# thu-ml/SageAttention

Measured on AMD Instinct MI355X. Metric: attention TFLOPS (causal, hd=128), kernel-only, as published by the reference, higher is better.
Workload: dtype int8 QK^T + fp8(e4m3) PV, fp32 accumulate

## Files before the change

sageattention_amd/csrc/sage_attn_kernel.h:

```cpp
#pragma once
#include "sage_common.h"
#include "sage_kernels.h"
#include "sage_attn_parts.h"
#include "sage_quant_math.h"
#include "sage_work_order.h"
#include <atomic>
#include <climits>
#include <cstdlib>
#include <type_traits>

#ifndef SAGE_ABL
#define SAGE_ABL 0
#endif
#ifndef SAGE_DIAG_PIPE
#define SAGE_DIAG_PIPE 1
#endif
#ifndef SAGE_KARG_PREFETCH
#define SAGE_KARG_PREFETCH 1
#endif
#ifndef SAGE_TAIL_PIPE
#define SAGE_TAIL_PIPE 1
#endif
#ifndef SAGE_KSEL
#define SAGE_KSEL 1
#endif
#ifndef SAGE_ATTN_TRACE
#define SAGE_ATTN_TRACE 0
#endif

#define SAGE_MIN_WAVES(D, MASK) ((MASK) != 0 ? 2 : ((D) == 64 ? 3 : 2))

#define SAGE_SCALE2_FOLD(d0, d1, s0, s1, c0, c1, m) "v_fma_f32 " d0 ", " s0 ", " c0 ", -" m "\n\tv_fma_f32 " d1 ", " s1 ", " c1 ", -" m "\n\t"
#define SAGE_SCALE2_EXACT(d0, d1, s0, s1, c0, c1, m) "v_add_f32 " d0 ", 0xbe22f983, " s0 "\n\tv_add_f32 " d1 ", 0xbe22f983, " s1 "\n\t" \
                                                      "v_fma_f32 " d0 ", " d0 ", " c0 ", -" m "\n\tv_fma_f32 " d1 ", " d1 ", " c1 ", -" m "\n\t"

#define SAGE_RENAME_S() do { const v4i z4_ = {0, 0, 0, 0};                                                                   \
        asm volatile("s_nop 15\n\ts_nop 7\n\tv_mfma_i32_32x32x32_i8 %0, %2, %2, %3\n\tv_mfma_i32_32x32x32_i8 %1, %2, %2, %4\n\t"     \
                     "s_nop 15\n\ts_nop 7" : "=&v"(sA[0]), "=&v"(sA[1]) : "v"(z4_), "v"(sB[0]), "v"(sB[1])); } while (0)

namespace sage {

constexpr int kHwregModeFp16Ovfl = 1 | (23 << 6) | (0 << 11);


template <int D, bool PV_FP8, int NH> struct TileCfg {
    static constexpr int KT = BLKK * NH;
    static constexpr int K_TILE_BYTES = KT * D;
    static constexpr int V_ROW_BYTES = PV_FP8 ? 64 : 128;
    static constexpr int V_IMG_BYTES = D * V_ROW_BYTES;
    static constexpr int STAGE_BYTES = K_TILE_BYTES + NH * V_IMG_BYTES;
    static constexpr int O_BYTES = BLKQ * D * 2;
    static constexpr int NSTAGE = 3;
    static constexpr int LDS_BYTES = (NSTAGE * STAGE_BYTES > O_BYTES) ? NSTAGE * STAGE_BYTES : O_BYTES;
    static constexpr int KSTEPS = D / 32;
    static constexpr int DT = D / 32;
};

__device__ __forceinline__ int crow(int r, int g) { return (r & 3) + 8 * (r >> 2) + 4 * g; }

constexpr int kSUnitLog2 = 26;
__device__ __forceinline__ float sfl(int x) { return __int_as_float(x) - __int_as_float(0x3E22F983); }
__device__ __forceinline__ v16i mfma_i8_first(v4i a, v4i b)
{
    v16i d;
    asm("s_nop 1\n\tv_mfma_i32_32x32x32_i8 %0, %1, %2, 0x3e22f983" : "=&v"(d) : "v"(a), "v"(b));
    return d;
}

#if SAGE_ATTN_TRACE
#define SAGE_TSTAMP(i) do { if (wave == 0) { unsigned long long t_; \
    asm volatile("s_memrealtime %0\n\ts_waitcnt lgkmcnt(0)" : "=s"(t_) :: "memory"); ttrace[i] = (unsigned)t_; } } while (0)
#else
#define SAGE_TSTAMP(i) do { } while (0)
#endif

template <int D, bool PV_FP8, bool CAUSAL, bool KTHREAD, bool TWO_LEVEL, int NH, int MASK = 0, int QF = 0, bool SFOLD = true, bool CPERS = false,
          bool VROWS = false, bool SEED = false>
__global__ void __launch_bounds__(256, SAGE_MIN_WAVES(D, MASK))
sage_attn_kernel(const AttnParams p_arg)
{
    typedef const __attribute__((address_space(4))) AttnParams *kparams_t;
    const kparams_t kp0 = (kparams_t)__builtin_amdgcn_kernarg_segment_ptr();
    const __attribute__((address_space(4))) AttnParams &p = *kp0;
    (void)p_arg;
#if SAGE_KARG_PREFETCH
    static_assert(sizeof(AttnParams) > 0x180, "prefetch offsets lie inside the parameter block");
    {
        unsigned t0, t1, t2, t3, t4, t5, t6;
        asm volatile("s_load_dword %0, %7, 0x0\n\ts_load_dword %1, %7, 0x40\n\ts_load_dword %2, %7, 0x80\n\ts_load_dword %3, %7, 0xc0\n\t"
                     "s_load_dword %4, %7, 0x100\n\ts_load_dword %5, %7, 0x140\n\ts_load_dword %6, %7, 0x180\n\ts_waitcnt lgkmcnt(0)"
                     : "=&s"(t0), "=&s"(t1), "=&s"(t2), "=&s"(t3), "=&s"(t4), "=&s"(t5), "=&s"(t6) : "s"(kp0) : "memory");
    }
#endif
    using C = TileCfg<D, PV_FP8, NH>;
    constexpr int KT = C::KT;
    constexpr int NS = 2 * NH;
    static_assert(!SEED || (PV_FP8 && KTHREAD && TWO_LEVEL && !SFOLD && MASK == 0 && (QF == 1 || QF == 2) && !CPERS && !VROWS),
                  "the seeded split: FP8 PV, fused per-thread Q, exact score form, dense");
    extern __shared__ __attribute__((aligned(16))) unsigned char smem[];

    const int wave_s = __builtin_amdgcn_readfirstlane((int)threadIdx.x >> 6);
#if SAGE_ATTN_TRACE
    __shared__ unsigned ttrace[16];
#endif
    constexpr bool PERS_OK = (!CAUSAL || CPERS) && MASK == 0;
    const bool pers = PERS_OK && p.sched != nullptr;
    __shared__ int s_ticket[2];
    int tpar = 0;
    int bid = blockIdx.x;
    unsigned next_k_v = 0;
    bool have_next = false, own_empty = false;
    auto kpl = [&]() -> kparams_t { kparams_t k = kp0; asm volatile("" : "+s"(k)); return k; };
    auto my_queue = [&]() -> int { return 4 * (int)(__builtin_amdgcn_s_getreg((3 << 11) | 20) & 7u) + (int)((blockIdx.x >> 3) & 3u); };
    auto logical_grid = [&]() -> int {
        const __attribute__((address_space(4))) AttnParams &pl = *kpl();
        int n = pl.nwg;
        if (pl.cu_q != nullptr && pl.work_items != nullptr) {
            typedef const __attribute__((address_space(4))) int *cint_p;
            const cint_p hdr = (cint_p)pl.work_hdr;
            n = 8 * (hdr[3] * ((hdr[0] + 7) >> 3) + (pl.Hq >> 3) * hdr[0]);
        }
        return n;
    };
    auto resolve_ticket = [&]() -> int {
        const int nwg_l = logical_grid();
        const int sched_first = gridDim.x >> 5;
        const int my_q = my_queue(), my_xcd = my_q >> 2;
        unsigned *const sched = kpl()->sched;
        if (have_next) {
            have_next = false;
            const int i = 32 * ((int)__builtin_amdgcn_readfirstlane(next_k_v) + sched_first) + 8 * (my_q & 3) + my_xcd;
            if (i < nwg_l) return i;
            own_empty = true;
        }
        int lane_o = (int)__builtin_amdgcn_mbcnt_hi(~0u, __builtin_amdgcn_mbcnt_lo(~0u, 0u));
        asm volatile("" : "+v"(lane_o));
        for (int attempt = 0; attempt < 4; attempt++) {
            const int q = lane_o & 31, x = q >> 2, s8x = 8 * (q & 3) + x;
            const unsigned c = lane_o < 32 ? __hip_atomic_load(sched + 32 * q, __ATOMIC_RELAXED, __HIP_MEMORY_SCOPE_AGENT) : 0u;
            const int cnt = nwg_l > s8x ? (nwg_l - s8x + 31) >> 5 : 0;
            int left = cnt - sched_first - (int)c;
            left = left < (1 << 24) ? left : (1 << 24) - 1;
            unsigned key = (lane_o < 32 && left > 0) ? ((x == my_xcd ? 1u : 0u) << 30) | ((unsigned)left << 5) | (unsigned)q : 0u;
#pragma unroll
            for (int m = 32; m >= 1; m >>= 1) { const unsigned o = __shfl_xor(key, m); key = o > key ? o : key; }
            key = __builtin_amdgcn_readfirstlane(key);
            if (key == 0u) return -1;
            const int bq = (int)(key & 31u);
            unsigned kv = 0;
            if (lane_o == 0) kv = __hip_atomic_fetch_add(sched + 32 * bq, 1u, __ATOMIC_RELAXED, __HIP_MEMORY_SCOPE_AGENT);
            const int i = 32 * ((int)__builtin_amdgcn_readfirstlane(kv) + sched_first) + 8 * (bq & 3) + (bq >> 2);
            if (i < nwg_l) return i;
        }
        return -1;
    };
    while (bid >= 0) {
    next_k_v = 0;
    do {
    kparams_t kp = kp0;
    if constexpr (PERS_OK) asm volatile("" : "+s"(kp));
    const __attribute__((address_space(4))) AttnParams &p = *kp;
    int lane_v = (int)__builtin_amdgcn_mbcnt_hi(~0u, __builtin_amdgcn_mbcnt_lo(~0u, 0u));
    if constexpr (PERS_OK) asm volatile("v_mbcnt_lo_u32_b32 %0, -1, 0\n\tv_mbcnt_hi_u32_b32 %0, -1, %0" : "=v"(lane_v));
    const int lane = lane_v;
    const int wave = wave_s;
    [[maybe_unused]] const int tid = wave * 64 + lane;
    int n = lane & 31;
    int g = lane >> 5;
    SAGE_TSTAMP(0);
    __builtin_amdgcn_s_setreg(kHwregModeFp16Ovfl, 1);

    const int nqblk = p.nqblk;
    int b, h, hk, qblk;
    if (p.cu_q != nullptr && p.work_items != nullptr) {
        typedef const __attribute__((address_space(4))) int *cint_p;
        const cint_p hdr = (cint_p)p.work_hdr;
        const int nitems = hdr[0];
        const WorkOrder wo = {hdr[1], hdr[2], hdr[3]};
        const int nwg = 8 * (wo.left * ((nitems + 7) >> 3) + (p.Hq >> 3) * nitems);
        int qrank;
        if (bid >= nwg || !work_item(wo, bid, nwg, p.Hq, nitems, h, qrank)) break;
        const cint_p items = (cint_p)p.work_items;
        b = items[2 * qrank];
        qblk = items[2 * qrank + 1];
        hk = h / p.group;
    } else if (p.cu_q != nullptr) {
        const int xcd = bid & 7, idx = bid >> 3;
        const int per_unit = nqblk * p.group;
        const int j = idx / per_unit, within = idx - j * per_unit;
        const int u = j * 8 + xcd;
        if (u >= p.B * p.Hkv) break;
        const int r = within / p.group, hg = within - r * p.group;
        qblk = nqblk - 1 - r;
        const int bs = u / p.Hkv;
        hk = u - bs * p.Hkv;
        b = p.seq_order != nullptr ? p.seq_order[bs] : bs;
        h = hk * p.group + hg;
    } else {
        int bh, qrank;
        const WorkOrder wo = {CAUSAL ? p.order_group : 0, p.order_fold, p.order_left};
        if (!work_item(wo, bid, pers ? p.nwg : (int)gridDim.x, p.B * p.Hq, nqblk, bh, qrank)) break;
        qblk = nqblk - 1 - qrank;
        b = bh / p.Hq;
        h = bh - b * p.Hq;
        hk = h / p.group;
    }

    int Lq = p.Lq, Lk = p.Lk;
    long q_off, k_off, o_off;
    long v_tile0, v_tstride;
    const float *qs_ptr, *ks_ptr;
    int qs_stride, ks_tstride;
    if (p.cu_q != nullptr) {
        typedef const __attribute__((address_space(4))) int *cint_p;
        const int bu = __builtin_amdgcn_readfirstlane(b);
        const int q0 = ((cint_p)p.cu_q)[bu], k0 = ((cint_p)p.cu_k)[bu], q1 = ((cint_p)p.cu_q)[bu + 1], k1 = ((cint_p)p.cu_k)[bu + 1];
        const int ks0 = ((cint_p)p.cu_ks)[bu];
        Lq = q1 - q0;
        Lk = k1 - k0;
        if (qblk * BLKQ >= Lq) break;
        q_off = (long)q0 * p.q_sl + (long)h * p.q_sh;
        k_off = (long)k0 * p.k_sl + (long)hk * p.k_sh;
        o_off = (long)q0 * p.o_sl + (long)h * p.o_sh;
        v_tile0 = (long)ks0 * p.Hkv + hk;
        v_tstride = p.Hkv;
        qs_ptr = QF == 0 ? p.q_scale + ((long)((cint_p)p.cu_qs)[bu] + qblk) * p.Hq + h : nullptr;
        qs_stride = 0;
        ks_ptr = p.k_scale + (long)ks0 * p.Hkv + hk;
        ks_tstride = p.Hkv;
    } else if constexpr (SEED) {
        const int hk0 = hk / p.kv_split, kc0 = p.kv_base + (hk - hk0 * p.kv_split) * Lk;
        const long bh0 = (long)b * (p.Hkv / p.kv_split) + hk0;
        q_off = (long)b * p.q_sb + (long)(hk0 * p.group + (h - hk * p.group)) * p.q_sh;
        k_off = (long)b * p.k_sb + (long)hk0 * p.k_sh + (long)kc0 * p.k_sl;
        o_off = (long)b * p.o_sb + (long)h * p.o_sh;
        v_tile0 = bh0 * (p.nks >> 2) + (kc0 >> 6);
        v_tstride = 1;
        qs_ptr = nullptr;
        qs_stride = 0;
        ks_ptr = p.k_scale + bh0 * p.nks + (kc0 >> 6) * 4;
        ks_tstride = 4;
    } else {
        const int hq = p.kv_split > 1 ? (hk / p.kv_split) * p.group + (h - hk * p.group) : h;
        q_off = (long)b * p.q_sb + (long)hq * p.q_sh;
        k_off = (long)b * p.k_sb + (long)hk * p.k_sh;
        o_off = (long)b * p.o_sb + (long)h * p.o_sh;
        const int ntk = (Lk + BLKK - 1) / BLKK;
        v_tile0 = ((long)b * p.Hkv + hk) * ntk;
        v_tstride = 1;
        qs_ptr = p.q_scale + ((long)b * p.Hq + h) * p.nqs + (long)qblk * p.qs_per_blk;
        qs_stride = 1;
        ks_ptr = p.k_scale + ((long)b * p.Hkv + hk) * p.nks;
        ks_tstride = KTHREAD ? 4 : 1;
    }

    SAGE_TSTAMP(1);
    const int row0 = qblk * BLKQ + wave * 32;
    int my_row = row0 + n;
    const int kchunk0 = SEED ? (CAUSAL ? p.kv_base + (hk % p.kv_split) * Lk : 0)
                             : ((CAUSAL && p.kv_split > 1 && p.cu_q == nullptr) ? (hk % p.kv_split) * Lk : 0);
    const int crow0 = row0 - kchunk0;
    int cmy_row = my_row - kchunk0;
    const int ntk_all = (Lk + BLKK - 1) / BLKK;
    int n_iters = (Lk + KT - 1) / KT;
    if (CAUSAL) {
        int lim = (qblk * BLKQ + BLKQ - kchunk0 + KT - 1) / KT;
        lim = lim > 0 ? lim : 0;
        n_iters = lim < n_iters ? lim : n_iters;
    }

    v4i qf[C::KSTEPS];
    float qsc;
    const unsigned char *kbase = reinterpret_cast<const unsigned char *>(p.k) + k_off;
    static_assert(!VROWS || (!PV_FP8 && MASK == 0), "V rows in place: FP16 PV, unmasked, dense launches");
    const unsigned char *vbase = reinterpret_cast<const unsigned char *>(p.v) + (VROWS ? 2 * ((long)b * p.v_sb + (long)hk * p.v_sh) : 0L);
    constexpr int CPR = D / 16;
    constexpr int KP = C::K_TILE_BYTES / 1024, VP = C::V_IMG_BYTES / 1024;
    unsigned koff[KP / 4];
#pragma unroll
    for (int i = 0; i < KP / 4; i++) {
        const int e = (wave * (KP / 4) + i) * 64 + lane;
        const int row = e / CPR, phys = e % CPR;
        koff[i] = (unsigned)(row * (int)p.k_sl + swz_chunk<D>(row, phys) * 16);
    }
    constexpr int CPRV = D / 8;
    constexpr int RPP = 64 / CPRV;
    [[maybe_unused]] unsigned voffr = 0;
    if constexpr (VROWS) {
        const int row = lane / CPRV, phys = lane % CPRV;
        const int logical = D == 128 ? (phys ^ ((row & 3) << 2)) : phys;
        voffr = (unsigned)(row * (int)p.v_sl * 2 + logical * 16);
    }
    typedef __attribute__((address_space(3))) unsigned char *lds_bytes;
    [[maybe_unused]] int vr_off[C::DT];
    if constexpr (VROWS) {
        const int s16 = lane & 15, hgrp = (lane >> 4) & 1;
#pragma unroll
        for (int dt = 0; dt < C::DT; dt++)
            vr_off[dt] = (4 * g + (s16 >> 2)) * (D * 2) + (D == 128 ? (dt ^ (s16 >> 2)) : dt) * 64 + 32 * hgrp + 8 * (s16 & 3);
    }
    auto v_frag = [&](const unsigned char *vs, int dt, int c) -> v4i {
        if constexpr (VROWS) {
            typedef short v4s __attribute__((ext_vector_type(4)));
            typedef short v8s __attribute__((ext_vector_type(8)));
            typedef __attribute__((address_space(3))) v4s *lds_v4s;
            const lds_bytes a0 = (lds_bytes)vs + vr_off[dt];
            const v4s lo = __builtin_amdgcn_ds_read_tr16_b64_v4i16((lds_v4s)(a0 + 16 * c * (D * 2)));
            const v4s hi = __builtin_amdgcn_ds_read_tr16_b64_v4i16((lds_v4s)(a0 + (16 * c + 8) * (D * 2)));
            return __builtin_bit_cast(v4i, (v8s)__builtin_shufflevector(lo, hi, 0, 1, 2, 3, 4, 5, 6, 7));
        } else {
            const int drow = dt * 32 + n;
            return *reinterpret_cast<const v4i *>(vs + drow * 128 + swz_chunk<128>(drow, 4 * g + c) * 16);
        }
    };
    int lane_g = lane;
    auto issue_loads = [&](int it, int buf) {
        unsigned char *ks = smem + buf * C::STAGE_BYTES;
        unsigned char *vs = ks + C::K_TILE_BYTES;
        const unsigned char *kt = kbase + (long)it * KT * p.k_sl;
        if (it * KT + KT <= Lk) {
#pragma unroll
            for (int i = 0; i < KP / 4; i++) {
                const int pc = wave * (KP / 4) + i;
                __builtin_amdgcn_global_load_lds((const __attribute__((address_space(1))) void *)(kt + koff[i]),
                                                 (__attribute__((address_space(3))) void *)(ks + pc * 1024), 16, 0, 0);
            }
        } else {
#pragma unroll
            for (int i = 0; i < KP / 4; i++) {
                const int pc = wave * (KP / 4) + i;
                const int e = pc * 64 + lane_g;
                const int row = e / CPR, phys = e % CPR;
                int key = it * KT + row;
                key = key < Lk ? key : Lk - 1;
                const unsigned char *src = kbase + (long)key * p.k_sl + swz_chunk<D>(row, phys) * 16;
                __builtin_amdgcn_global_load_lds((const __attribute__((address_space(1))) void *)src,
                                                 (__attribute__((address_space(3))) void *)(ks + pc * 1024), 16, 0, 0);
            }
        }
#pragma unroll
        for (int hh = 0; hh < NH; hh++) {
            int tv = it * NH + hh;
            tv = tv < ntk_all ? tv : ntk_all - 1;
            if constexpr (VROWS) {
#pragma unroll
                for (int i = 0; i < VP / 4; i++) {
                    const int pc = wave * (VP / 4) + i;
                    int tok = tv * BLKK + pc * RPP + lane_g / CPRV;
                    tok = tok < Lk ? tok : Lk - 1;
                    const int row = pc * RPP + lane_g / CPRV, phys = lane_g % CPRV;
                    const int logical = D == 128 ? (phys ^ ((row & 3) << 2)) : phys;
                    __builtin_amdgcn_global_load_lds((const __attribute__((address_space(1))) void *)(vbase + (long)tok * p.v_sl * 2 + logical * 16),
                                                     (__attribute__((address_space(3))) void *)(vs + hh * C::V_IMG_BYTES + pc * 1024), 16, 0, 0);
                }
            } else {
            const unsigned char *vt = vbase + (v_tile0 + (long)tv * v_tstride) * (long)C::V_IMG_BYTES;
#pragma unroll
            for (int i = 0; i < VP / 4; i++) {
                const int pc = wave * (VP / 4) + i;
                __builtin_amdgcn_global_load_lds((const __attribute__((address_space(1))) void *)(vt + pc * 1024 + lane_g * 16),
                                                 (__attribute__((address_space(3))) void *)(vs + hh * C::V_IMG_BYTES + pc * 1024), 16, 0, 0);
            }
            }
        }
    };

    v16f o[C::DT];
#pragma unroll
    for (int dt = 0; dt < C::DT; dt++)
#pragma unroll
        for (int i = 0; i < 16; i++) o[dt][i] = 0.0f;
    float m_run = kNegBig, l_run = 0.0f;
    constexpr float OFF = PV_FP8 ? kFp8Offset : 0.0f;

    typedef const __attribute__((address_space(4))) float *cfloat_p;
    const cfloat_p ks_c = (cfloat_p)(ks_ptr);
    float ksc[NH][2];
    auto load_kscales = [&](int it, float (&dst)[NH][2]) {
#pragma unroll
        for (int hh = 0; hh < NH; hh++) {
            int tk = it * NH + hh;
            tk = tk < ntk_all ? tk : ntk_all - 1;
            const long tb = (long)(tk >> p.ks_shift) * ks_tstride;
            if (KTHREAD) {
                const float s0 = ks_c[tb], s1 = ks_c[tb + 1], s2 = ks_c[tb + 2], s3 = ks_c[tb + 3];
                dst[hh][0] = g ? s2 : s0;
                dst[hh][1] = g ? s3 : s1;
            } else {
                dst[hh][0] = dst[hh][1] = ks_c[tb];
            }
        }
    };
    constexpr int NSTAGE = C::NSTAGE;
    constexpr int DMA_PER_TILE = KP / 4 + NH * (VP / 4);
    auto ring_wait = [&](bool younger_in_flight) {
        if (younger_in_flight) asm volatile("s_waitcnt vmcnt(%0)" ::"n"(DMA_PER_TILE) : "memory");
        else asm volatile("s_waitcnt vmcnt(0)" ::: "memory");
        __builtin_amdgcn_s_barrier();
    };
    if (n_iters > 0) {
        load_kscales(0, ksc);
        issue_loads(0, 0);
    }
    if (n_iters > 1) issue_loads(1, 1);
    if constexpr (QF == 0) {
        const int8_t *qrow = reinterpret_cast<const int8_t *>(p.q) + q_off + (long)my_row * p.q_sl;
        const bool ok = my_row < Lq;
#pragma unroll
        for (int ks = 0; ks < C::KSTEPS; ks++) {
            v4i z = {0, 0, 0, 0};
            qf[ks] = ok ? *reinterpret_cast<const v4i *>(qrow + 32 * ks + 16 * g) : z;
        }
        int slot;
        const int rin = wave * 32 + n;
        if (p.q_gran == QG_PER_BLOCK) slot = 0;
        else if (p.q_gran == QG_PER_WARP32) slot = rin >> 5;
        else if (p.q_gran == QG_PER_WARP16) slot = rin >> 4;
        else if (p.q_gran == QG_PER_THREAD16) slot = (rin >> 4) * 8 + (rin & 7);
        else slot = (rin >> 5) * 8 + (rin & 7);
        qsc = qs_ptr[slot * qs_stride];
    } else {
        constexpr int QDT = (QF == 1 || QF == 3) ? DT_F16 : DT_BF16;
        constexpr bool QBLOCK = QF >= 3;
        const float premul = QBLOCK ? p.q_premul : 1.0f;
        const uint16_t *qrow = reinterpret_cast<const uint16_t *>(p.q) + q_off + (long)my_row * p.q_sl;
        const bool ok = my_row < Lq;
        float x[C::KSTEPS][16];
        float amax = 0.0f;
#pragma unroll
        for (int ks = 0; ks < C::KSTEPS; ks++) {
            v4u raw[2] = {{0u, 0u, 0u, 0u}, {0u, 0u, 0u, 0u}};
            if (ok) {
                raw[0] = *reinterpret_cast<const v4u *>(qrow + 32 * ks + 16 * g);
                raw[1] = *reinterpret_cast<const v4u *>(qrow + 32 * ks + 16 * g + 8);
            }
#pragma unroll
            for (int j = 0; j < 16; j++) {
                const unsigned w = raw[j >> 3][(j & 7) >> 1];
                float f = ld16<QDT>((uint16_t)((j & 1) ? (w >> 16) : (w & 0xffffu)));
                if constexpr (QBLOCK) f *= premul;
                x[ks][j] = f;
                amax = fmaxf(amax, fabsf(f));
            }
        }
        if constexpr (QBLOCK) {
            amax = fmaxf(amax, __shfl_xor(amax, 1));
            amax = fmaxf(amax, __shfl_xor(amax, 2));
            amax = fmaxf(amax, __shfl_xor(amax, 4));
        }
        amax = fmaxf(amax, __shfl_xor(amax, 8));
        amax = fmaxf(amax, __shfl_xor(amax, 16));
        amax = fmaxf(amax, __shfl_xor(amax, 32));
        if constexpr (QBLOCK) {
            __shared__ float q_amax[4];
            if (lane == 0) q_amax[wave] = amax;
            asm volatile("s_waitcnt lgkmcnt(0)" ::: "memory");
            __builtin_amdgcn_s_barrier();
            amax = fmaxf(fmaxf(q_amax[0], q_amax[1]), fmaxf(q_amax[2], q_amax[3]));
        }
        const float sc = quant_scale(amax, QBLOCK ? QS_TRITON : QS_TRITON_THREAD);
        const float y = quant_recip(sc);
        qsc = sc;
#pragma unroll
        for (int ks = 0; ks < C::KSTEPS; ks++) {
            int q8[16];
#pragma unroll
            for (int j = 0; j < 16; j++) q8[j] = QBLOCK ? quant_round_triton(x[ks][j], sc, y) : quant_round_triton_nz(x[ks][j], sc, y);
#pragma unroll
            for (int w = 0; w < 4; w++) qf[ks][w] = (int)pack_int8x4(q8[4 * w], q8[4 * w + 1], q8[4 * w + 2], q8[4 * w + 3]);
        }
    }

    if constexpr (SEED) {
        if (my_row < Lq) {
            const int hk0 = hk / p.kv_split;
            const long gl = (long)p.group * Lq;
            const float *sm = p.seed_max + ((long)b * (p.Hkv / p.kv_split) + hk0) * p.seed_chunks * gl + (long)(h - hk * p.group) * Lq + my_row;
            const int c_end = p.seed_first + (hk - hk0 * p.kv_split);
            for (int c = 0; c < c_end; c++) m_run = fmaxf(m_run, sm[c * gl]);
        }
    }
    SAGE_TSTAMP(2);
    ring_wait(n_iters > 1);
    SAGE_TSTAMP(3);

    int cur = 0;
    auto tile_iter = [&](const int it) {
        const bool more = (it + 1) < n_iters;
        const bool more2 = (it + 2) < n_iters;
        const int nxt = (cur + 1 == NSTAGE) ? 0 : cur + 1;
        float ksc_next[NH][2];
        if (more) load_kscales(it + 1, ksc_next);
        if (more2) issue_loads(it + 2, (nxt + 1 == NSTAGE) ? 0 : nxt + 1);

        int nact = 0;
#pragma unroll
        for (int hh = 0; hh < NH; hh++) {
            const int key0 = it * KT + hh * BLKK;
            if (key0 < Lk && (!CAUSAL || key0 <= crow0 + 31)) nact = hh + 1;
        }
        float mk[MASK ? NS : 1][16];
        bool skip_tile = false;
        if constexpr (MASK != 0) {
            const unsigned char *mbase = reinterpret_cast<const unsigned char *>(p.mask);
            const long mrow = (long)b * p.m_sb + (long)h * p.m_sh + (long)my_row * p.m_sq;
            int anytrue = 0;
#pragma unroll
            for (int sb = 0; sb < NS; sb++)
#pragma unroll
                for (int i = 0; i < 16; i++) {
                    const int key = it * KT + sb * 32 + crow(i, g);
                    const bool inb = (my_row < Lq) && (key < Lk);
                    float add = -1.0e6f;
                    if (inb) {
                        const long idx = mrow + (long)key * p.m_sk;
                        if (MASK == 1) { const bool t = mbase[idx] != 0; add = t ? 0.0f : -1.0e6f; anytrue |= (int)t; }
                        else if (MASK == 2) add = f16_to_f32(reinterpret_cast<const uint16_t *>(mbase)[idx]);
                        else add = bf16_to_f32(reinterpret_cast<const uint16_t *>(mbase)[idx]);
                    }
                    mk[sb][i] = add;
                }
            if (MASK == 1) skip_tile = !__syncthreads_or(anytrue);
        }
        if (nact > 0 && !skip_tile) {
            const unsigned char *ks = smem + cur * C::STAGE_BYTES;
            const unsigned char *vs = ks + C::K_TILE_BYTES;
            const int last_key = it * KT + nact * BLKK - 1;
            const bool full = (MASK == 0) && (nact == NH) && !(CAUSAL && last_key > crow0) && (last_key < Lk);

            v16i s[NS];
#pragma unroll
            for (int sb = 0; sb < NS; sb++) {
#pragma unroll
                for (int i = 0; i < 16; i++) s[sb][i] = 0;
                if (sb < 2 * nact) {
                    const int krow = sb * 32 + n;
#pragma unroll
                    for (int kk = 0; kk < C::KSTEPS; kk++) {
                        const v4i a = *reinterpret_cast<const v4i *>(ks + krow * D + swz_chunk<D>(krow, 2 * kk + g) * 16);
                        s[sb] = kk == 0 ? mfma_i8_first(a, qf[kk]) : __builtin_amdgcn_mfma_i32_32x32x32_i8(a, qf[kk], s[sb], 0, 0, 0);
                    }
                }
            }

            float cs[NH][2];
#pragma unroll
            for (int hh = 0; hh < NH; hh++) {
                cs[hh][0] = __builtin_ldexpf(p.sm_scale_log2 * (qsc * ksc[hh][0]), kSUnitLog2);
                cs[hh][1] = KTHREAD ? __builtin_ldexpf(p.sm_scale_log2 * (qsc * ksc[hh][1]), kSUnitLog2) : cs[hh][0];
            }

            float m_new;
            if (full) {
                float mxc = -INFINITY;
#pragma unroll
                for (int hh = 0; hh < NH; hh++) {
                    int mx0 = INT_MIN, mx1 = INT_MIN;
#pragma unroll
                    for (int u = 0; u < 2; u++)
#pragma unroll
                        for (int i = 0; i < 16; i++) {
                            if (KTHREAD && (i & 2)) mx1 = max(mx1, s[2 * hh + u][i]);
                            else mx0 = max(mx0, s[2 * hh + u][i]);
                        }
                    mxc = fmaxf(mxc, __builtin_fmaf(sfl(mx0), cs[hh][0], -OFF));
                    if (KTHREAD) mxc = fmaxf(mxc, __builtin_fmaf(sfl(mx1), cs[hh][1], -OFF));
                }
                m_new = fmaxf(m_run, pair_max(mxc));
            } else {
                float mx = -INFINITY;
#pragma unroll
                for (int sb = 0; sb < NS; sb++)
#pragma unroll
                    for (int i = 0; i < 16; i++) {
                        if (sb < 2 * nact) {
                            const float cc = cs[sb >> 1][(KTHREAD && (i & 2)) ? 1 : 0];
                            const int key = it * KT + sb * 32 + crow(i, g);
                            const bool ok = (key < Lk) && (!CAUSAL || key <= cmy_row);
                            if constexpr (MASK != 0) mx = fmaxf(mx, (ok ? sfl(s[sb][i]) * cc : 0.0f) + mk[sb][i] - OFF);
                            else mx = fmaxf(mx, ok ? __builtin_fmaf(sfl(s[sb][i]), cc, -OFF) : -INFINITY);
                        }
                    }
                m_new = fmaxf(m_run, pair_max(mx));
            }
            const float alpha = __builtin_amdgcn_exp2f(m_run - m_new);
            m_run = m_new;
            if (!TWO_LEVEL) {
#pragma unroll
                for (int dt = 0; dt < C::DT; dt++)
#pragma unroll
                    for (int i = 0; i < 16; i++) o[dt][i] *= alpha;
            }

            constexpr bool sum_rounded = !PV_FP8 && !TWO_LEVEL;
            constexpr bool GFOLD = PV_FP8 && SFOLD && MASK == 0;
            float rs = 0.0f;
            auto p_chunk = [&](auto masked, auto rnd, int hh, int c, float (&e)[8]) {
                const int sb = 2 * hh + (c >> 1), r0 = (c & 1) * 8;
                [[maybe_unused]] const float mbf0 = GFOLD ? __builtin_fmaf(__int_as_float(0x3E22F983), cs[hh][0], m_new) : 0.0f;
                [[maybe_unused]] const float mbf1 = (GFOLD && KTHREAD) ? __builtin_fmaf(__int_as_float(0x3E22F983), cs[hh][1], m_new) : mbf0;
#pragma unroll
                for (int j = 0; j < 8; j++) {
                    const int i = r0 + j;
                    const float cc = cs[hh][(KTHREAD && (i & 2)) ? 1 : 0];
                    float v;
                    if constexpr (MASK != 0) {
                        const int key = it * KT + sb * 32 + crow(i, g);
                        v = __builtin_amdgcn_exp2f(((key < Lk) ? sfl(s[sb][i]) * cc : 0.0f) + mk[sb][i] - m_new);
                    } else {
                        if constexpr (GFOLD) v = __builtin_amdgcn_exp2f(__builtin_fmaf(__int_as_float(s[sb][i]), cc, -((KTHREAD && (i & 2)) ? mbf1 : mbf0)));
                        else v = __builtin_amdgcn_exp2f(__builtin_fmaf(sfl(s[sb][i]), cc, -m_new));
                        if constexpr (decltype(masked)::value) {
                            const int key = it * KT + sb * 32 + crow(i, g);
                            const bool ok = (sb < 2 * nact) && (key < Lk) && (!CAUSAL || key <= cmy_row);
                            v = ok ? v : 0.0f;
                        }
                    }
                    e[j] = v;
                    if constexpr (decltype(rnd)::value) rs += (float)(_Float16)v;
                    else rs += v;
                }
            };

            if constexpr (PV_FP8) {
                int pw[NH][8];
                auto build_p = [&](auto masked) {
#pragma unroll
                    for (int hh = 0; hh < NH; hh++)
#pragma unroll
                        for (int c = 0; c < 4; c++) {
                            float e[8];
                            p_chunk(masked, std::false_type{}, hh, c, e);
                            int w0 = __builtin_amdgcn_cvt_pk_fp8_f32(e[0], e[1], __float_as_int(e[0]), false);
                            w0 = __builtin_amdgcn_cvt_pk_fp8_f32(e[2], e[3], w0, true);
                            int w1 = __builtin_amdgcn_cvt_pk_fp8_f32(e[4], e[5], __float_as_int(e[4]), false);
                            w1 = __builtin_amdgcn_cvt_pk_fp8_f32(e[6], e[7], w1, true);
                            pw[hh][2 * c] = w0;
                            pw[hh][2 * c + 1] = w1;
                        }
                };
                if (full) build_p(std::false_type{});
                else build_p(std::true_type{});
                l_run = l_run * alpha + rs;
                auto pv = [&](auto fold_tag) {
                    constexpr bool FOLD = decltype(fold_tag)::value;
#pragma unroll
                    for (int dt = 0; dt < C::DT; dt++) {
                        const int drow = dt * 32 + n;
                        v16f acc;
                        if (FOLD) {
#pragma unroll
                            for (int i = 0; i < 16; i++) acc[i] = 0.0f;
                        } else acc = o[dt];
#pragma unroll
                        for (int hh = 0; hh < NH; hh++) {
                            if (hh < nact) {
                                const unsigned char *vr = vs + hh * C::V_IMG_BYTES + drow * 64;
                                const v4u va = *reinterpret_cast<const v4u *>(vr + swz_chunk<64>(drow, 2 * g) * 16);
                                const v4u vb = *reinterpret_cast<const v4u *>(vr + swz_chunk<64>(drow, 2 * g + 1) * 16);
                                const v8i av = {(int)va[0], (int)va[1], (int)va[2], (int)va[3], (int)vb[0], (int)vb[1], (int)vb[2], (int)vb[3]};
                                const v8i bv = {pw[hh][0], pw[hh][1], pw[hh][2], pw[hh][3], pw[hh][4], pw[hh][5], pw[hh][6], pw[hh][7]};
                                acc = __builtin_amdgcn_mfma_scale_f32_32x32x64_f8f6f4(av, bv, acc, 0, 0, 0, 0, 0, 0);
                            }
                        }
                        if (FOLD) {
#pragma unroll
                            for (int i = 0; i < 16; i++) o[dt][i] = __builtin_fmaf(o[dt][i], alpha, acc[i]);
                        } else o[dt] = acc;
                    }
                };
                if constexpr (!TWO_LEVEL) pv(std::false_type{});
                else pv(std::true_type{});
            } else {
                v8h pb[NH][4];
                auto build_p = [&](auto masked, auto rnd) {
#pragma unroll
                    for (int hh = 0; hh < NH; hh++)
#pragma unroll
                        for (int c = 0; c < 4; c++) {
                            float e[8];
                            p_chunk(masked, rnd, hh, c, e);
#pragma unroll
                            for (int j = 0; j < 8; j++) pb[hh][c][j] = (_Float16)e[j];
                        }
                };
                if (full) build_p(std::false_type{}, std::integral_constant<bool, sum_rounded>{});
                else build_p(std::true_type{}, std::integral_constant<bool, sum_rounded>{});
                l_run = l_run * alpha + rs;
                auto pv = [&](auto fold_tag) {
                    constexpr bool FOLD = decltype(fold_tag)::value;
#pragma unroll
                    for (int dt = 0; dt < C::DT; dt++) {
                        v16f acc;
                        if (FOLD) {
#pragma unroll
                            for (int i = 0; i < 16; i++) acc[i] = 0.0f;
                        } else acc = o[dt];
#pragma unroll
                        for (int hh = 0; hh < NH; hh++) {
                            if (hh < nact) {
#pragma unroll
                                for (int c = 0; c < 4; c++) {
                                    const v8h a = __builtin_bit_cast(v8h, v_frag(vs + hh * C::V_IMG_BYTES, dt, c));
                                    acc = __builtin_amdgcn_mfma_f32_32x32x16_f16(a, pb[hh][c], acc, 0, 0, 0);
                                }
                            }
                        }
                        if (FOLD) {
#pragma unroll
                            for (int i = 0; i < 16; i++) o[dt][i] = __builtin_fmaf(o[dt][i], alpha, acc[i]);
                        } else o[dt] = acc;
                    }
                };
                if constexpr (!TWO_LEVEL) pv(std::false_type{});
                else pv(std::true_type{});
            }
        }

        if (more) {
#pragma unroll
            for (int hh = 0; hh < NH; hh++) { ksc[hh][0] = ksc_next[hh][0]; ksc[hh][1] = ksc_next[hh][1]; }
        }
        ring_wait(more2);
        cur = nxt;
    };

    int it = 0;
    if constexpr (MASK == 0) {
        static_assert(NH == 1 && NSTAGE == 3, "the pipelined loops are written for 64-key iterations on the 3-slot ring");
        constexpr bool SIX_BODIES = D == 128 || PV_FP8;
        int n_steady = Lk / KT - 2;
        n_steady = n_steady < n_iters - 2 ? n_steady : n_iters - 2;
        if (CAUSAL) {
            int nd = (qblk * BLKQ - kchunk0) / KT;
            nd = nd > 0 ? nd : 0;
            n_steady = n_steady < nd ? n_steady : nd;
        }
        constexpr bool DIAG_PIPE = CAUSAL && SAGE_DIAG_PIPE && (PV_FP8 || D == 128);
        const bool diag_ok = DIAG_PIPE && (n_steady > 0 ? n_iters - n_steady == 2 : (PV_FP8 && n_iters == 2 && Lk >= 2 * KT));
        constexpr bool TAIL_PIPE = !CAUSAL && SAGE_TAIL_PIPE && (PV_FP8 || D == 128);
        const bool tail_ok = TAIL_PIPE && n_steady == Lk / KT - 2 &&
                             (PV_FP8 ? (n_steady >= 0 && n_iters - n_steady <= (SAGE_TAIL_PIPE == 2 ? 2 : 3)) : (n_steady > 0 && n_iters - n_steady == 2));

        if constexpr (PV_FP8) {
#include "sage_attn_loop_f8.h"
        } else {
#include "sage_attn_loop_f16.h"
        }
    }
    if constexpr (MASK == 0) {
        asm volatile("v_mbcnt_lo_u32_b32 %0, -1, 0\n\tv_mbcnt_hi_u32_b32 %0, -1, %0" : "=v"(lane_g));
        n = lane_g & 31;
        g = lane_g >> 5;
        my_row = row0 + n;
        cmy_row = my_row - kchunk0;
    }
#pragma nounroll
    for (; it < n_iters; it++) tile_iter(it);
    SAGE_TSTAMP(4);
    __syncthreads();
    SAGE_TSTAMP(5);
    if (pers && !own_empty) {
        if (wave == 0 && lane_g == 0) next_k_v = __hip_atomic_fetch_add(kpl()->sched + 32 * my_queue(), 1u, __ATOMIC_RELAXED, __HIP_MEMORY_SCOPE_AGENT);
        have_next = true;
    }

    __builtin_amdgcn_s_setreg(kHwregModeFp16Ovfl, 0);
    const float l_tot = pair_sum(l_run);
    const float inv = l_tot > 0.0f ? __builtin_amdgcn_rcpf(l_tot) : 0.0f;
    if (p.lse != nullptr && g == 0 && my_row < Lq) {
        long lidx = (p.cu_q != nullptr) ? ((long)h * p.lse_sh + p.cu_q[b] + my_row)
                                        : ((long)b * p.Hq + h) * (long)p.Lq + my_row;
        p.lse[lidx] = __builtin_amdgcn_logf(l_tot) + m_run;
    }
    unsigned char *obuf = smem + wave * (32 * D * 2);
    const long vbh = SEED ? (long)b * (p.Hkv / p.kv_split) + hk / p.kv_split : (long)b * p.Hkv + hk;
    const float *vsc = PV_FP8 ? p.v_scale + vbh * D : nullptr;
    const float *vmn = (p.v_mean != nullptr) ? p.v_mean + vbh * D : nullptr;
    v4f sc4[C::DT][4], mn4[C::DT][4];
#pragma unroll
    for (int dt = 0; dt < C::DT; dt++) {
#pragma unroll
        for (int r4 = 0; r4 < 4; r4++) {
            const v4f one = {1.0f, 1.0f, 1.0f, 1.0f};
            sc4[dt][r4] = PV_FP8 ? *reinterpret_cast<const v4f *>(vsc + dt * 32 + 8 * r4 + 4 * g) : one;
        }
        if (vmn != nullptr) {
#pragma unroll
            for (int r4 = 0; r4 < 4; r4++) mn4[dt][r4] = *reinterpret_cast<const v4f *>(vmn + dt * 32 + 8 * r4 + 4 * g);
        } else {
#pragma unroll
            for (int r4 = 0; r4 < 4; r4++) { const v4f z = {0.0f, 0.0f, 0.0f, 0.0f}; mn4[dt][r4] = z; }
        }
    }
#pragma unroll
    for (int dt = 0; dt < C::DT; dt++) {
#pragma unroll
        for (int r4 = 0; r4 < 4; r4++) {
            const int d0 = dt * 32 + 8 * r4 + 4 * g;
            float x[4];
#pragma unroll
            for (int j = 0; j < 4; j++) {
                x[j] = o[dt][4 * r4 + j] * inv;
                if (PV_FP8) x[j] *= sc4[dt][r4][j];
                x[j] += mn4[dt][r4][j];
            }
            if constexpr (SEED) {
                if (my_row < Lq) *reinterpret_cast<v4f *>(reinterpret_cast<float *>(p.o) + o_off + (long)my_row * p.o_sl + d0) = v4f{x[0], x[1], x[2], x[3]};
                continue;
            }
            v2u pk;
            if (p.out_dtype == DT_F16) {
                pk[0] = (unsigned)f32_to_f16_rne(x[0]) | ((unsigned)f32_to_f16_rne(x[1]) << 16);
                pk[1] = (unsigned)f32_to_f16_rne(x[2]) | ((unsigned)f32_to_f16_rne(x[3]) << 16);
            } else {
                pk[0] = (unsigned)f32_to_bf16_rne(x[0]) | ((unsigned)f32_to_bf16_rne(x[1]) << 16);
                pk[1] = (unsigned)f32_to_bf16_rne(x[2]) | ((unsigned)f32_to_bf16_rne(x[3]) << 16);
            }
            const int q8 = d0 >> 2;
            const int Q = (q8 >> 1) ^ (n & 7);
            *reinterpret_cast<v2u *>(obuf + n * (D * 2) + Q * 16 + (q8 & 1) * 8) = pk;
        }
    }
    asm volatile("s_waitcnt lgkmcnt(0)" ::: "memory");
    if constexpr (!SEED) {
        constexpr int LPR = D * 2 / 16;
        constexpr int RPP = 64 / LPR;
        unsigned char *obase = reinterpret_cast<unsigned char *>(p.o) + 2 * o_off;
#pragma unroll
        for (int pass = 0; pass < 32 / RPP; pass++) {
            const int r = pass * RPP + lane_g / LPR, Q = lane_g % LPR;
            const v4u val = *reinterpret_cast<const v4u *>(obuf + r * (D * 2) + (Q ^ (r & 7)) * 16);
            const int grow = row0 + r;
            if (grow < Lq) *reinterpret_cast<v4u *>(obase + 2 * ((long)grow * p.o_sl) + Q * 16) = val;
        }
    }
#if SAGE_ATTN_TRACE
    SAGE_TSTAMP(6);
    asm volatile("s_waitcnt vmcnt(0)" ::: "memory");
    SAGE_TSTAMP(7);
    if (wave == 0 && p.trace != nullptr && bid < p.trace_wgs) {
        if (lane < 8 || lane == 8 || lane >= 13) p.trace[16 * bid + lane] = ttrace[lane];
        if (lane == 9) p.trace[16 * bid + 9] = __builtin_amdgcn_s_getreg((31 << 11) | 4);
        if (lane == 10) p.trace[16 * bid + 10] = __builtin_amdgcn_s_getreg((31 << 11) | 20);
        if (lane == 11) p.trace[16 * bid + 11] = blockIdx.x;
        if (lane == 12) p.trace[16 * bid + 12] = (unsigned)qblk;
    }
#endif
    } while (0);
    if (!pers) break;
    if (wave_s == 0) { const int t = resolve_ticket(); if (__builtin_amdgcn_mbcnt_hi(~0u, __builtin_amdgcn_mbcnt_lo(~0u, 0u)) == 0) s_ticket[tpar] = t; }
    __syncthreads();
    bid = __builtin_amdgcn_readfirstlane(s_ticket[tpar]);
    tpar ^= 1;
    }
    if constexpr (PERS_OK) {
        if (pers && wave_s == 0) {
            unsigned *const sched = kpl()->sched;
            const int lane_x = (int)__builtin_amdgcn_mbcnt_hi(~0u, __builtin_amdgcn_mbcnt_lo(~0u, 0u));
            unsigned gone = 0;
            if (lane_x == 0) gone = __hip_atomic_fetch_add(sched + kAttnSchedDoneWord, 1u, __ATOMIC_ACQ_REL, __HIP_MEMORY_SCOPE_AGENT);
            if ((unsigned)__builtin_amdgcn_readfirstlane(gone) + 1u == gridDim.x) {
                if (lane_x < 32) __hip_atomic_store(sched + 32 * lane_x, 0u, __ATOMIC_RELAXED, __HIP_MEMORY_SCOPE_AGENT);
                if (lane_x == 32) __hip_atomic_store(sched + kAttnSchedDoneWord, 0u, __ATOMIC_RELAXED, __HIP_MEMORY_SCOPE_AGENT);
            }
        }
    }
}

}
```

sageattention_amd/csrc/sage_common.h:

```cpp
#pragma once
#include <hip/hip_runtime.h>
#include <stdint.h>

namespace sage {

typedef int v4i __attribute__((ext_vector_type(4)));
typedef int v8i __attribute__((ext_vector_type(8)));
typedef int v16i __attribute__((ext_vector_type(16)));
typedef float v16f __attribute__((ext_vector_type(16)));
typedef float v4f __attribute__((ext_vector_type(4)));
typedef float v2f __attribute__((ext_vector_type(2)));
typedef _Float16 v8h __attribute__((ext_vector_type(8)));
typedef _Float16 v2h __attribute__((ext_vector_type(2)));
typedef unsigned int v4u __attribute__((ext_vector_type(4)));
typedef unsigned int v2u __attribute__((ext_vector_type(2)));

constexpr int kWave = 64;
constexpr int BLKQ = 128;
constexpr int BLKK = 64;
constexpr float kFp8Offset = 8.807f;
constexpr float kNegBig = -1.0e30f;

enum : int { DT_F16 = 0, DT_BF16 = 1 };

__host__ __device__ inline int pv_token_of_position(int p)
{
    const int g = p >> 5, c = (p >> 3) & 3, j = p & 7;
    return 16 * c + 8 * (j >> 2) + 4 * g + (j & 3);
}

template <int ROW_BYTES>
__host__ __device__ inline int swz_chunk(int row, int chunk)
{
    if constexpr (ROW_BYTES == 128) return chunk ^ ((row >> 1) & 7);
    else if constexpr (ROW_BYTES == 64) return chunk ^ ((row >> 2) & 3);
    else return chunk;
}

__device__ inline float bf16_to_f32(uint16_t b) { return __uint_as_float(((uint32_t)b) << 16); }
__device__ inline uint16_t f32_to_bf16_rne(float f)
{
    uint32_t x = __float_as_uint(f);
    x += 0x7fffu + ((x >> 16) & 1u);
    return (uint16_t)(x >> 16);
}
__device__ inline float f16_to_f32(uint16_t h)
{
    _Float16 v; __builtin_memcpy(&v, &h, 2); return (float)v;
}
__device__ inline uint16_t f32_to_f16_rne(float f)
{
    _Float16 v = (_Float16)f; uint16_t h; __builtin_memcpy(&h, &v, 2); return h;
}
template <int DT> __device__ inline float ld16(uint16_t raw)
{
    if constexpr (DT == DT_F16) return f16_to_f32(raw); else return bf16_to_f32(raw);
}
template <int DT> __device__ inline uint16_t st16(float f)
{
    if constexpr (DT == DT_F16) return f32_to_f16_rne(f); else return f32_to_bf16_rne(f);
}

__device__ inline float pair_max(float x)
{
    auto r = __builtin_amdgcn_permlane32_swap(__float_as_uint(x), __float_as_uint(x), false, false);
    return fmaxf(__uint_as_float(r[0]), __uint_as_float(r[1]));
}
__device__ inline float pair_sum(float x)
{
    auto r = __builtin_amdgcn_permlane32_swap(__float_as_uint(x), __float_as_uint(x), false, false);
    return __uint_as_float(r[0]) + __uint_as_float(r[1]);
}

template <typename IntPtr>
__device__ __forceinline__ void varlen_segment(IntPtr cu, int nseq, int total, int seg, int &t0, int &len)
{
    if (seg < nseq) { t0 = cu[seg]; len = cu[seg + 1] - t0; }
    else if (seg == nseq) { t0 = cu[nseq]; len = total - t0; }
    else { t0 = 0; len = cu[0]; }
    len = len > 0 ? len : 0;
}

}
```

Measured before the change: 1604.

## Trim attention epilogue: prefetch scale factors before barrier, specialize output conversion and stores

Issues the v_scale/v_mean loads before the end-of-loop barrier so their latency overlaps the wait, and replaces __syncthreads with a raw s_barrier. The output conversion is specialized by dtype at compile time, with bf16 using a packed hardware conversion. The global store loop batches its LDS reads and skips per-row bounds checks when the whole tile is in range. The gains are limited to the per-tile epilogue, and the packed bf16 conversion may round differently from the manual RNE on NaN inputs.

```diff
diff --git a/sageattention_amd/csrc/sage_attn_kernel.h b/sageattention_amd/csrc/sage_attn_kernel.h
--- a/sageattention_amd/csrc/sage_attn_kernel.h
+++ b/sageattention_amd/csrc/sage_attn_kernel.h
@@ -23,6 +23,9 @@
 #endif
 #ifndef SAGE_KSEL
 #define SAGE_KSEL 1
+#endif
+#ifndef SAGE_ITEM_TRIM
+#define SAGE_ITEM_TRIM 2
 #endif
 #ifndef SAGE_ATTN_TRACE
 #define SAGE_ATTN_TRACE 0
@@ -758,7 +761,36 @@
 #pragma nounroll
     for (; it < n_iters; it++) tile_iter(it);
     SAGE_TSTAMP(4);
-    __syncthreads();
+    constexpr bool TRIM_EPI = (SAGE_ITEM_TRIM & 2) != 0;
+    const long vbh = SEED ? (long)b * (p.Hkv / p.kv_split) + hk / p.kv_split : (long)b * p.Hkv + hk;
+    const float *vsc = PV_FP8 ? p.v_scale + vbh * D : nullptr;
+    const float *vmn = (p.v_mean != nullptr) ? p.v_mean + vbh * D : nullptr;
+    v4f sc4[C::DT][4], mn4[C::DT][4];
+    auto load_factors = [&]() {
+#pragma unroll
+        for (int dt = 0; dt < C::DT; dt++) {
+#pragma unroll
+            for (int r4 = 0; r4 < 4; r4++) {
+                const v4f one = {1.0f, 1.0f, 1.0f, 1.0f};
+                sc4[dt][r4] = PV_FP8 ? *reinterpret_cast<const v4f *>(vsc + dt * 32 + 8 * r4 + 4 * g) : one;
+            }
+            if (vmn != nullptr) {
+#pragma unroll
+                for (int r4 = 0; r4 < 4; r4++) mn4[dt][r4] = *reinterpret_cast<const v4f *>(vmn + dt * 32 + 8 * r4 + 4 * g);
+            } else {
+#pragma unroll
+                for (int r4 = 0; r4 < 4; r4++) { const v4f z = {0.0f, 0.0f, 0.0f, 0.0f}; mn4[dt][r4] = z; }
+            }
+        }
+    };
+    if constexpr (TRIM_EPI) {
+        load_factors();
+        asm volatile("s_waitcnt lgkmcnt(0)" ::: "memory");
+        __builtin_amdgcn_s_barrier();
+        asm volatile("" ::: "memory");
+    } else {
+        __syncthreads();
+    }
     SAGE_TSTAMP(5);
     if (pers && !own_empty) {
         if (wave == 0 && lane_g == 0) next_k_v = __hip_atomic_fetch_add(kpl()->sched + 32 * my_queue(), 1u, __ATOMIC_RELAXED, __HIP_MEMORY_SCOPE_AGENT);
@@ -774,65 +806,75 @@
         p.lse[lidx] = __builtin_amdgcn_logf(l_tot) + m_run;
     }
     unsigned char *obuf = smem + wave * (32 * D * 2);
-    const long vbh = SEED ? (long)b * (p.Hkv / p.kv_split) + hk / p.kv_split : (long)b * p.Hkv + hk;
-    const float *vsc = PV_FP8 ? p.v_scale + vbh * D : nullptr;
-    const float *vmn = (p.v_mean != nullptr) ? p.v_mean + vbh * D : nullptr;
-    v4f sc4[C::DT][4], mn4[C::DT][4];
-#pragma unroll
-    for (int dt = 0; dt < C::DT; dt++) {
-#pragma unroll
-        for (int r4 = 0; r4 < 4; r4++) {
-            const v4f one = {1.0f, 1.0f, 1.0f, 1.0f};
-            sc4[dt][r4] = PV_FP8 ? *reinterpret_cast<const v4f *>(vsc + dt * 32 + 8 * r4 + 4 * g) : one;
-        }
-        if (vmn != nullptr) {
-#pragma unroll
-            for (int r4 = 0; r4 < 4; r4++) mn4[dt][r4] = *reinterpret_cast<const v4f *>(vmn + dt * 32 + 8 * r4 + 4 * g);
-        } else {
-#pragma unroll
-            for (int r4 = 0; r4 < 4; r4++) { const v4f z = {0.0f, 0.0f, 0.0f, 0.0f}; mn4[dt][r4] = z; }
-        }
-    }
-#pragma unroll
-    for (int dt = 0; dt < C::DT; dt++) {
-#pragma unroll
-        for (int r4 = 0; r4 < 4; r4++) {
-            const int d0 = dt * 32 + 8 * r4 + 4 * g;
-            float x[4];
-#pragma unroll
-            for (int j = 0; j < 4; j++) {
-                x[j] = o[dt][4 * r4 + j] * inv;
-                if (PV_FP8) x[j] *= sc4[dt][r4][j];
-                x[j] += mn4[dt][r4][j];
-            }
-            if constexpr (SEED) {
-                if (my_row < Lq) *reinterpret_cast<v4f *>(reinterpret_cast<float *>(p.o) + o_off + (long)my_row * p.o_sl + d0) = v4f{x[0], x[1], x[2], x[3]};
-                continue;
-            }
-            v2u pk;
-            if (p.out_dtype == DT_F16) {
-                pk[0] = (unsigned)f32_to_f16_rne(x[0]) | ((unsigned)f32_to_f16_rne(x[1]) << 16);
-                pk[1] = (unsigned)f32_to_f16_rne(x[2]) | ((unsigned)f32_to_f16_rne(x[3]) << 16);
-            } else {
-                pk[0] = (unsigned)f32_to_bf16_rne(x[0]) | ((unsigned)f32_to_bf16_rne(x[1]) << 16);
-                pk[1] = (unsigned)f32_to_bf16_rne(x[2]) | ((unsigned)f32_to_bf16_rne(x[3]) << 16);
-            }
-            const int q8 = d0 >> 2;
-            const int Q = (q8 >> 1) ^ (n & 7);
-            *reinterpret_cast<v2u *>(obuf + n * (D * 2) + Q * 16 + (q8 & 1) * 8) = pk;
-        }
-    }
+    if constexpr (!TRIM_EPI) load_factors();
+    auto convert_rows = [&](auto dtype) {
+        constexpr int DTYPE = decltype(dtype)::value;
+#pragma unroll
+        for (int dt = 0; dt < C::DT; dt++) {
+#pragma unroll
+            for (int r4 = 0; r4 < 4; r4++) {
+                const int d0 = dt * 32 + 8 * r4 + 4 * g;
+                float x[4];
+#pragma unroll
+                for (int j = 0; j < 4; j++) {
+                    x[j] = o[dt][4 * r4 + j] * inv;
+                    if (PV_FP8) x[j] *= sc4[dt][r4][j];
+                    x[j] += mn4[dt][r4][j];
+                }
+                if constexpr (SEED) {
+                    if (my_row < Lq) *reinterpret_cast<v4f *>(reinterpret_cast<float *>(p.o) + o_off + (long)my_row * p.o_sl + d0) = v4f{x[0], x[1], x[2], x[3]};
+                    continue;
+                }
+                v2u pk;
+                if (DTYPE == DT_F16 || (DTYPE < 0 && p.out_dtype == DT_F16)) {
+                    pk[0] = (unsigned)f32_to_f16_rne(x[0]) | ((unsigned)f32_to_f16_rne(x[1]) << 16);
+                    pk[1] = (unsigned)f32_to_f16_rne(x[2]) | ((unsigned)f32_to_f16_rne(x[3]) << 16);
+                } else if constexpr (DTYPE < 0) {
+                    pk[0] = (unsigned)f32_to_bf16_rne(x[0]) | ((unsigned)f32_to_bf16_rne(x[1]) << 16);
+                    pk[1] = (unsigned)f32_to_bf16_rne(x[2]) | ((unsigned)f32_to_bf16_rne(x[3]) << 16);
+                } else {
+                    pk[0] = f32x2_to_bf16x2(x[0], x[1]);
+                    pk[1] = f32x2_to_bf16x2(x[2], x[3]);
+                }
+                const int q8 = d0 >> 2;
+                const int Q = (q8 >> 1) ^ (n & 7);
+                *reinterpret_cast<v2u *>(obuf + n * (D * 2) + Q * 16 + (q8 & 1) * 8) = pk;
+            }
+        }
+    };
+    if constexpr (SEED || !TRIM_EPI) convert_rows(std::integral_constant<int, -1>{});
+    else if (p.out_dtype == DT_F16) convert_rows(std::integral_constant<int, DT_F16>{});
+    else convert_rows(std::integral_constant<int, DT_BF16>{});
     asm volatile("s_waitcnt lgkmcnt(0)" ::: "memory");
     if constexpr (!SEED) {
         constexpr int LPR = D * 2 / 16;
         constexpr int RPP = 64 / LPR;
         unsigned char *obase = reinterpret_cast<unsigned char *>(p.o) + 2 * o_off;
-#pragma unroll
-        for (int pass = 0; pass < 32 / RPP; pass++) {
-            const int r = pass * RPP + lane_g / LPR, Q = lane_g % LPR;
-            const v4u val = *reinterpret_cast<const v4u *>(obuf + r * (D * 2) + (Q ^ (r & 7)) * 16);
-            const int grow = row0 + r;
-            if (grow < Lq) *reinterpret_cast<v4u *>(obase + 2 * ((long)grow * p.o_sl) + Q * 16) = val;
+        if constexpr (TRIM_EPI) {
+            const int r0 = lane_g / LPR, Q = lane_g % LPR;
+            unsigned char *const dst = obase + 2 * ((long)(row0 + r0) * p.o_sl) + Q * 16;
+            const long step = 2 * (long)RPP * p.o_sl;
+            v4u val[32 / RPP];
+#pragma unroll
+            for (int pass = 0; pass < 32 / RPP; pass++) {
+                const int r = pass * RPP + r0;
+                val[pass] = *reinterpret_cast<const v4u *>(obuf + r * (D * 2) + (Q ^ (r & 7)) * 16);
+            }
+            auto store_rows = [&](auto whole) {
+#pragma unroll
+                for (int pass = 0; pass < 32 / RPP; pass++)
+                    if (decltype(whole)::value || row0 + pass * RPP + r0 < Lq) *reinterpret_cast<v4u *>(dst + pass * step) = val[pass];
+            };
+            if (row0 + 31 < Lq) store_rows(std::true_type{});
+            else store_rows(std::false_type{});
+        } else {
+#pragma unroll
+            for (int pass = 0; pass < 32 / RPP; pass++) {
+                const int r = pass * RPP + lane_g / LPR, Q = lane_g % LPR;
+                const v4u val = *reinterpret_cast<const v4u *>(obuf + r * (D * 2) + (Q ^ (r & 7)) * 16);
+                const int grow = row0 + r;
+                if (grow < Lq) *reinterpret_cast<v4u *>(obase + 2 * ((long)grow * p.o_sl) + Q * 16) = val;
+            }
         }
     }
 #if SAGE_ATTN_TRACE
diff --git a/sageattention_amd/csrc/sage_common.h b/sageattention_amd/csrc/sage_common.h
--- a/sageattention_amd/csrc/sage_common.h
+++ b/sageattention_amd/csrc/sage_common.h
@@ -44,6 +44,13 @@
     x += 0x7fffu + ((x >> 16) & 1u);
     return (uint16_t)(x >> 16);
 }
+__device__ inline uint32_t f32x2_to_bf16x2(float x, float y)
+{
+    typedef float v2f_ __attribute__((ext_vector_type(2)));
+    typedef __bf16 v2bf_ __attribute__((ext_vector_type(2)));
+    const v2f_ f = {x, y};
+    return __builtin_bit_cast(uint32_t, __builtin_convertvector(f, v2bf_));
+}
 __device__ inline float f16_to_f32(uint16_t h)
 {
     _Float16 v; __builtin_memcpy(&v, &h, 2); return (float)v;
```

Result: no change. 1615, median of 6 (+0.7%).
